# GestaltCogTeam/STEP

Measured on AMD Instinct MI355X. Metric: training windows/sec on PEMS04, horizon-12 MAE parity, 1/2/4/8 MI355X, higher is better.
Workload: dtype f16 (TSFormer Q/K/weights) + bf16 (P, V, GraphWaveNet / graph-learner GEMMs) operands, f32 accumulate

## Files before the change

include/step_hip.h:

```cpp
#ifndef STEP_HIP_H
#define STEP_HIP_H

#include <stdint.h>

#ifdef __cplusplus
extern "C" {
#endif

const char* step_last_error(void);
int step_abi_version(void);

typedef struct StepGemm {
    int M, N, K, batch;
    const void* A; long sam, sak, sab; int a_bf16;
    const void* B; long sbk, sbn, sbb; int b_bf16;
    float* C; long ldc, scn, scb;
    float alpha;
    int accumulate;
    const float* bias; int relu;
    int splitk;
    int a_kblk; long a_kstride;
    int b_kblk; long b_kstride;
    int b_nblk; long b_nstride;
    int c_nblk; long c_nstride;
// ... 8 lines not shown
int step_gemm(const StepGemm* g, void* stream);

#define STEP_ENC_F16 1
#define STEP_ENC_ALWAYS_RESHIFT 2
#define STEP_ENC_RANGE_FLAG 4
#define STEP_ENC_WORKGROUPS(n) (((n) & 0xffff) << 8)
int step_tsformer_encode(const float* series, int S, int L, const void* wpack, long wpack_bytes,
                         int depth, int flags, uint16_t* hidden_bf16, float* hidden_f32, float* last_f32,
                         float* sqnorm_part, float dropout_p, const uint64_t* drop_pool, long pool_words, uint64_t seed,
                         unsigned int* fallback_count, void* stream);
int step_dropout_pool_fill(uint64_t* pool, long words, float dropout_p, uint64_t seed, void* stream);
long step_tsformer_dropout_words(int L, int depth);

int step_pack_long_history(const float* x, int B, int L, int N, int C, int ch, float* out, void* stream);
int step_gather_windows(const float* data, int T, int N, int C, int ch, const long* t0, int B, int L, int H,
                        float* long_series, float* hist, float* fut, void* stream);

long step_knn_workspace_bytes(int B, int N, int F);
int step_knn_graph(const uint16_t* hidden, const float* sqnorm_part, int B, int N, int F, int k_total,
                   float* sim, float* adj, void* work, long work_bytes, void* stream);
int step_topk_mask(const float* sim, int B, int N, int k_total, float* adj, void* work, long work_bytes,
                   void* stream);

typedef struct StepDglParams {
    float *conv1_w, *conv1_b;
    float *conv2_w, *conv2_b;
    float *fc_w, *fc_b;
    float *bn1_w, *bn1_b, *bn1_rm, *bn1_rv;
    float *bn2_w, *bn2_b, *bn2_rm, *bn2_rv;
    float *bn3_w, *bn3_b, *bn3_rm, *bn3_rv;
    float *fc_out_w, *fc_out_b;
    float *fc_cat_w, *fc_cat_b;
    int gemm_bf16;
} StepDglParams;

long step_dgl_global_saved_floats(int N, int T);
long step_dgl_global_work_floats(int N, int T, int backward);
int step_dgl_global_forward(const float* series_nt, int N, int T, const StepDglParams* p, int training,
                            float momentum, float* saved, float* work, float* g, void* stream);
int step_dgl_global_backward(const float* series_nt, int N, int T, const StepDglParams* p, const float* saved,
                             const float* dg, float* work, const StepDglParams* grads, void* stream);
#define STEP_DGL_FRESH_FC_GRAD 16
int step_dgl_global_backward_phase(const float* series_nt, int N, int T, const StepDglParams* p, const float* saved,
                             const float* dg, float* work, const StepDglParams* grads, int phase, void* stream);

typedef struct StepDglShard { int own1; double count1, count2; } StepDglShard;
int step_dgl_global_forward_shard(const float* series_slice, int N, int Ts, const StepDglParams* p, int training, float momentum,
                                  float* saved, float* work, double* sums, float* g, const StepDglShard* shard, int phase,
                                  void* stream);
int step_dgl_global_backward_shard(const float* series_slice, int N, int Ts, const StepDglParams* p, const float* saved,
                                   const float* dg, float* work, const StepDglParams* grads, const StepDglShard* shard, int phase,
                                   void* stream);
long step_dgl_global_offset(int N, int T, int item);

long step_dgl_edges_saved_floats(int B, int N);
long step_dgl_edges_work_floats(int N);
long step_dgl_edges_theta_offset(int N);
int step_dgl_edges_forward(const float* g, int N, int B, const StepDglParams* p, const float* u, uint64_t seed,
                           float temperature, float* saved, float* theta_out, float* adj_out, void* stream);
int step_dgl_edges_forward_keyed(const float* g, int N, int B, const StepDglParams* p, const long* key, uint64_t seed,
                                 float temperature, float* saved, float* theta_out, float* adj_out, void* stream);
int step_dgl_edges_backward(const float* g, int N, int B, const StepDglParams* p, const float* saved,
                            const float* dtheta, const float* dadj, float temperature, float* work,
                            const StepDglParams* grads, float* dg, void* aux_stream, void* stream);
int step_dgl_edges_backward_acc(const float* g, int N, int B, const StepDglParams* p, const float* saved,
                                const float* dtheta, const float* dadj, float temperature, float* work,
                                const StepDglParams* grads, float* dg, int dg_accumulate, void* aux_stream, void* stream);

typedef struct StepGwnetParams {
    float *nodevec1, *nodevec2;
    float *start_w, *start_b;
    float *filter_w[8], *filter_b[8];
    float *gate_w[8], *gate_b[8];
    float *skip_w[8], *skip_b[8];
    float *bn_w[8], *bn_b[8], *bn_rm[8], *bn_rv[8];
    float *gconv_w[8], *gconv_b[8];
    float *fc_his0_w, *fc_his0_b, *fc_his2_w, *fc_his2_b;
    float *end1_w, *end1_b, *end2_w, *end2_b;
    int gemm_bf16;
} StepGwnetParams;

long step_gwnet_saved_floats(int B, int N, int dropout);
long step_gwnet_work_floats(int B, int N, int backward);
long step_gwnet_saved_offset(int B, int N, int dropout, int item, int layer);
int step_gwnet_forward(const float* hist, int B, int N, int Cin, const float* hidden_last, const float* adj,
                       const StepGwnetParams* p, int training, float dropout_p, uint64_t seed, float momentum,
                       float* saved, float* work, float* pred, void* stream);
int step_gwnet_forward_phase(const float* hist, int B, int N, int Cin, const float* hidden_last, const float* adj,
                             const StepGwnetParams* p, int training, float dropout_p, uint64_t seed, float momentum,
                             float* saved, float* work, float* pred, int phase, void* stream);
int step_gwnet_backward(const float* hist, int B, int N, int Cin, const float* hidden_last, const StepGwnetParams* p,
                        const float* saved, float* work, const float* dpred, const StepGwnetParams* grads,
                        float* dadj, int dropout, void* aux_stream, void* leaf_stream, void* stream);

int step_pt_dropout(const float* x, float* y, long n, float p, uint64_t seed, uint32_t site, void* stream);
int step_pt_ffn_hidden_fwd(const float* x, const float* w1, const float* b1, long R, float p, uint64_t seed, uint32_t site,
                           uint16_t* hidden, void* stream);
int step_pt_ffn_hidden_bwd(const float* dy, const float* w2, const uint16_t* hidden, long R, float p, uint16_t* dhidden, void* stream);
int step_pt_colsum_bf16(const uint16_t* x, long rows, int cols, float* out, void* stream);
long step_pt_rows_linear_pack_bytes(int nkc, int nog);
int step_pt_rows_linear_pack(const float* w, long swo, long swi, int nkc, int nog, const float* bias, void* pack, void* stream);
int step_pt_rows_linear(const void* x, int x_bf16, long R, const void* pack, int nkc, int nog, void* y, int y_bf16, int accumulate, void* stream);
int step_pt_layer_pack(const float* wi, const float* bi, const float* wo, const float* bo, const float* w1, const float* b1, const float* w2,
                       const float* b2, void* ffn, void* qkv, void* o, void* da, void* dx, void* stream);
long step_pt_proj_wgrad_ws_floats(long R);
int step_pt_proj_wgrad(const float* x, const uint16_t* dqkv, const float* dov, const uint16_t* a, long R, float* ws, float* dwi, float* dbi, float* dwo,
// ... 141 lines not shown
```

step_amd/_lib.py:

```python
import ctypes
import os

import torch

_HERE = os.path.dirname(os.path.abspath(__file__))
LIB_PATH = os.environ.get("STEP_HIP_LIB") or os.path.join(_HERE, "libstep_hip.so")

_vp, _i, _l, _f, _u64 = ctypes.c_void_p, ctypes.c_int, ctypes.c_long, ctypes.c_float, ctypes.c_uint64


class StepGemm(ctypes.Structure):
    _fields_ = [("M", _i), ("N", _i), ("K", _i), ("batch", _i),
                ("A", _vp), ("sam", _l), ("sak", _l), ("sab", _l), ("a_bf16", _i),
                ("B", _vp), ("sbk", _l), ("sbn", _l), ("sbb", _l), ("b_bf16", _i),
                ("C", _vp), ("ldc", _l), ("scn", _l), ("scb", _l),
                ("alpha", _f), ("accumulate", _i), ("bias", _vp), ("relu", _i), ("splitk", _i),
                ("a_kblk", _i), ("a_kstride", _l), ("b_kblk", _i), ("b_kstride", _l),
                ("b_nblk", _i), ("b_nstride", _l), ("c_nblk", _i), ("c_nstride", _l),
                ("a_kscale", _vp), ("a_kshift", _vp), ("a_kperiod", _i),
                ("batch0", _i), ("sab1", _l), ("sbb1", _l), ("scb1", _l), ("compute_bf16", _i), ("a_rowsum", _vp), ("c_nscale", _vp), ("c_nshift", _vp), ("c_mvec", _vp),
                ("c_nperiod", _i), ("splitk_ws", _vp), ("splitk_ws_floats", _l)]


class StepDglParams(ctypes.Structure):
    NAMES = ["conv1_w", "conv1_b", "conv2_w", "conv2_b", "fc_w", "fc_b",
             "bn1_w", "bn1_b", "bn1_rm", "bn1_rv", "bn2_w", "bn2_b", "bn2_rm", "bn2_rv",
             "bn3_w", "bn3_b", "bn3_rm", "bn3_rv", "fc_out_w", "fc_out_b", "fc_cat_w", "fc_cat_b"]
    _fields_ = [(n, _vp) for n in NAMES] + [("gemm_bf16", _i)]


class StepGwnetParams(ctypes.Structure):
    _fields_ = [("nodevec1", _vp), ("nodevec2", _vp), ("start_w", _vp), ("start_b", _vp),
                ("filter_w", _vp * 8), ("filter_b", _vp * 8), ("gate_w", _vp * 8), ("gate_b", _vp * 8),
                ("skip_w", _vp * 8), ("skip_b", _vp * 8),
                ("bn_w", _vp * 8), ("bn_b", _vp * 8), ("bn_rm", _vp * 8), ("bn_rv", _vp * 8),
                ("gconv_w", _vp * 8), ("gconv_b", _vp * 8),
                ("fc_his0_w", _vp), ("fc_his0_b", _vp), ("fc_his2_w", _vp), ("fc_his2_b", _vp),
                ("end1_w", _vp), ("end1_b", _vp), ("end2_w", _vp), ("end2_b", _vp), ("gemm_bf16", _i)]


_PD = ctypes.POINTER(StepDglParams)


class StepDynState(ctypes.Structure):
    _fields_ = [("seed_xor", ctypes.c_uint64), ("adam_step", ctypes.c_int32), ("lr", _f), ("gsl_coef", _f), ("reserved", _f)]


class StepDglShard(ctypes.Structure):
    _fields_ = [("own1", ctypes.c_int), ("count1", ctypes.c_double), ("count2", ctypes.c_double)]


_PS = ctypes.POINTER(StepDglShard)
_PG = ctypes.POINTER(StepGwnetParams)

_SIGS = {
    "step_last_error": (ctypes.c_char_p, []),
    "step_abi_version": (_i, []),
    "step_gemm": (_i, [ctypes.POINTER(StepGemm), _vp]),
    "step_tsformer_encode": (_i, [_vp, _i, _i, _vp, _l, _i, _i, _vp, _vp, _vp, _vp, _f, _vp, _l, _u64, _vp, _vp]),
    "step_dropout_pool_fill": (_i, [_vp, _l, _f, _u64, _vp]),
    "step_tsformer_dropout_words": (_l, [_i, _i]),
    "step_gather_windows": (_i, [_vp, _i, _i, _i, _i, _vp, _i, _i, _i, _vp, _vp, _vp, _vp]),
    "step_pack_long_history": (_i, [_vp, _i, _i, _i, _i, _i, _vp, _vp]),
    "step_knn_workspace_bytes": (_l, [_i, _i, _i]),
    "step_knn_graph": (_i, [_vp, _vp, _i, _i, _i, _i, _vp, _vp, _vp, _l, _vp]),
    "step_topk_mask": (_i, [_vp, _i, _i, _i, _vp, _vp, _l, _vp]),
    "step_selftest_mfma": (_i, [_vp, _vp]),
    "step_streams_concurrent": (_i, [_vp, _vp, ctypes.POINTER(_i)]),
    "step_dgl_global_saved_floats": (_l, [_i, _i]),
    "step_dgl_global_work_floats": (_l, [_i, _i, _i]),
    "step_dgl_global_forward": (_i, [_vp, _i, _i, _PD, _i, _f, _vp, _vp, _vp, _vp]),
    "step_dgl_global_backward": (_i, [_vp, _i, _i, _PD, _vp, _vp, _vp, _PD, _vp]),
    "step_dgl_global_backward_phase": (_i, [_vp, _i, _i, _PD, _vp, _vp, _vp, _PD, _i, _vp]),
    "step_dgl_global_forward_shard": (_i, [_vp, _i, _i, _PD, _i, _f, _vp, _vp, _vp, _vp, _PS, _i, _vp]),
    "step_dgl_global_backward_shard": (_i, [_vp, _i, _i, _PD, _vp, _vp, _vp, _PD, _PS, _i, _vp]),
    "step_dgl_global_offset": (_l, [_i, _i, _i]),
    "step_dgl_edges_saved_floats": (_l, [_i, _i]),
    "step_dgl_edges_work_floats": (_l, [_i]),
    "step_dgl_edges_theta_offset": (_l, [_i]),
    "step_dgl_edges_forward": (_i, [_vp, _i, _i, _PD, _vp, _u64, _f, _vp, _vp, _vp, _vp]),
    "step_dgl_edges_forward_keyed": (_i, [_vp, _i, _i, _PD, _vp, _u64, _f, _vp, _vp, _vp, _vp]),
    "step_dgl_edges_backward": (_i, [_vp, _i, _i, _PD, _vp, _vp, _vp, _f, _vp, _PD, _vp, _vp, _vp]),
    "step_dgl_edges_backward_acc": (_i, [_vp, _i, _i, _PD, _vp, _vp, _vp, _f, _vp, _PD, _vp, _i, _vp, _vp]),
    "step_gwnet_saved_floats": (_l, [_i, _i, _i]),
    "step_gwnet_work_floats": (_l, [_i, _i, _i]),
    "step_gwnet_saved_offset": (_l, [_i, _i, _i, _i, _i]),
    "step_gwnet_forward": (_i, [_vp, _i, _i, _i, _vp, _vp, _PG, _i, _f, _u64, _f, _vp, _vp, _vp, _vp]),
    "step_gwnet_forward_phase": (_i, [_vp, _i, _i, _i, _vp, _vp, _PG, _i, _f, _u64, _f, _vp, _vp, _vp, _i, _vp]),
    "step_gwnet_backward": (_i, [_vp, _i, _i, _i, _vp, _PG, _vp, _vp, _vp, _PG, _vp, _i, _vp, _vp, _vp]),
    "step_pt_dropout": (_i, [_vp, _vp, _l, _f, _u64, ctypes.c_uint32, _vp]),
    "step_pt_ffn_hidden_fwd": (_i, [_vp, _vp, _vp, _l, _f, _u64, ctypes.c_uint32, _vp, _vp]),
    "step_pt_ffn_hidden_bwd": (_i, [_vp, _vp, _vp, _l, _f, _vp, _vp]),
    "step_pt_colsum_bf16": (_i, [_vp, _l, _i, _vp, _vp]),
    "step_pt_rows_linear_pack_bytes": (_l, [_i, _i]),
    "step_pt_rows_linear_pack": (_i, [_vp, _l, _l, _i, _i, _vp, _vp, _vp]),
    "step_pt_rows_linear": (_i, [_vp, _i, _l, _vp, _i, _i, _vp, _i, _i, _vp]),
    "step_pt_layer_pack": (_i, [_vp] * 14),
    "step_pt_proj_wgrad_ws_floats": (_l, [_l]),
    "step_pt_proj_wgrad": (_i, [_vp, _vp, _vp, _vp, _l, _vp, _vp, _vp, _vp, _vp]),
    "step_pt_ffn_fused_fwd_ln": (_i, [_vp, _l, _vp, _f, _vp, _l, _u64, ctypes.c_uint32, ctypes.c_uint32, _vp, _vp, _vp, _vp, _vp, _vp]),
    "step_pt_rows_linear_ln": (_i, [_vp, _l, _vp, _vp, _f, _u64, ctypes.c_uint32, _vp, _vp, _vp, _vp, _vp, _vp]),
    "step_pt_embed_unmasked_fwd": (_i, [_vp, _vp, _vp, _vp, _vp, _l, _i, _i, _f, _u64, ctypes.c_uint32, _vp, _vp]),
    "step_pt_embed_unmasked_bwd": (_i, [_vp, _vp, _vp, _l, _i, _i, _f, _u64, ctypes.c_uint32, _vp, _vp, _vp, _vp]),
    "step_pt_dec_input_bwd_sums": (_i, [_vp, _l, _i, _i, _f, _u64, ctypes.c_uint32, _vp, _vp, _vp, _vp, _vp]),
    "step_pt_ffn_pack_bytes": (_l, []),
    "step_pt_ffn_wgrad_workgroups": (_l, [_l]),
    "step_pt_ffn_wgrad_ws_floats": (_l, [_l]),
    "step_pt_ffn_pack": (_i, [_vp, _vp, _vp, _vp, _vp, _vp]),
    "step_pt_ffn_fused_fwd": (_i, [_vp, _l, _vp, _f, _vp, _l, _u64, ctypes.c_uint32, _vp, _vp]),
    "step_pt_ffn_fused_bwd_data": (_i, [_vp, _vp, _l, _vp, _f, _vp, _l, _u64, ctypes.c_uint32, _vp, _vp]),
    "step_pt_ffn_fused_bwd_weights": (_i, [_vp, _vp, _l, _vp, _vp, _f, _vp, _l, _u64, ctypes.c_uint32, _vp, _vp, _vp, _vp, _vp]),
    "step_pt_add_layernorm_fwd": (_i, [_vp, _vp, _l, _f, _u64, ctypes.c_uint32, _vp, _vp, _vp, _vp, _vp, _vp]),
    "step_pt_layernorm_bwd_dropout": (_i, [_vp, _vp, _l, _vp, _vp, _vp, _vp, _f, _u64, ctypes.c_uint32, _vp, _vp, _vp, _vp]),
    "step_pt_dropout_relu_mask": (_i, [_vp, _vp, _l, _f, _u64, ctypes.c_uint32, _vp]),
    "step_pt_add_dropout": (_i, [_vp, _vp, _vp, _l, _f, _u64, ctypes.c_uint32, _vp]),
    "step_pt_add_rows": (_i, [_vp, _l, _i, _vp, _vp, _vp]),
    "step_pt_sum_over_seq": (_i, [_vp, _l, _i, _i, _i, _vp, _vp, _vp]),
    "step_pt_token_gather": (_i, [_vp, _l, _i, _vp, _i, _f, _vp, _vp]),
    "step_pt_token_scatter": (_i, [_vp, _l, _i, _vp, _i, _f, _vp, _vp]),
    "step_pt_dec_input": (_i, [_vp, _vp, _vp, _vp, _l, _i, _i, _f, _u64, ctypes.c_uint32, _vp, _vp]),
    "step_pt_dec_input_bwd": (_i, [_vp, _l, _i, _i, _f, _u64, ctypes.c_uint32, _vp, _vp, _vp]),
    "step_pt_layernorm_fwd": (_i, [_vp, _l, _vp, _vp, _vp, _vp, _vp]),
    "step_pt_layernorm_bwd": (_i, [_vp, _vp, _l, _vp, _vp, _vp, _vp, _vp, _vp]),
    "step_pt_attention_fwd": (_i, [_vp, _l, _i, _f, _u64, ctypes.c_uint32, _vp, _vp, _vp]),
    "step_pt_attention_bwd": (_i, [_vp, _vp, _vp, _vp, _l, _i, _f, _u64, ctypes.c_uint32, _vp, _vp]),
    "step_pt_attention_fwd_bf16": (_i, [_vp, _l, _i, _f, _u64, ctypes.c_uint32, _vp, _vp, _vp, _vp, _l, _vp]),
    "step_pt_attention_bwd_bf16": (_i, [_vp, _vp, _vp, _vp, _l, _i, _f, _u64, ctypes.c_uint32, _vp, _vp, _vp]),
    "step_pt_linear_bf16out": (_i, [_vp, _vp, _l, _l, _vp, _l, _i, _i, _vp, _vp]),
    "step_pt_relu_mask": (_i, [_vp, _vp, _l, _vp]),
# ... 122 lines not shown
```

step_amd/csrc/dgl.hip:

```cpp
#include "common.h"
#include "step_internal.h"

namespace {

constexpr int KW = 10;
constexpr int EMB = 100;

template <int CI, int CO, int TPT>
__global__ __launch_bounds__(256) void conv_relu_fwd_kernel(const float* __restrict__ in, const float* __restrict__ w,
                                                            const float* __restrict__ b, const float* __restrict__ in_sc,
                                                            const float* __restrict__ in_sh, float* __restrict__ out,
                                                            float* __restrict__ partial, int Tin, int stat_limit) {
    __shared__ __attribute__((aligned(16))) float ws[CI * KW * CO];
    __shared__ float red[4][2 * CO];
    const int tid = threadIdx.x, n = blockIdx.y;
    const int Tout = Tin - (KW - 1);
    for (int e = tid; e < CI * KW * CO; e += 256) {
        int co = e % CO, k = (e / CO) % KW, ci = e / (CO * KW);
        ws[e] = w[(co * CI + ci) * KW + k];
    }
    __syncthreads();
    const int t0 = (blockIdx.x * 256 + tid) * TPT;
    float acc[CO][TPT];
#pragma unroll
// ... 622 lines not shown
    if (i < n) gpre[i] = shiftdot[i % EMB];
}
__global__ __launch_bounds__(256) void fc_unpermute_kernel(const float* __restrict__ graw, const float* __restrict__ fc_w,
                                                           const float* __restrict__ st2, const float* __restrict__ colsum,
                                                           float* __restrict__ dfc_w, float* __restrict__ dots_o, int T2, int overwrite) {
    __shared__ float red[16][32];
    const int o = blockIdx.y, t = blockIdx.x * 256 + threadIdx.x, tid = threadIdx.x, lane = tid & 63, wave = tid >> 6;
    const float cso = colsum[o];
    float d[32];
#pragma unroll
    for (int i = 0; i < 32; ++i) d[i] = 0.f;
    if (t < T2) {
        const float4* src = (const float4*)(graw + ((long)o * T2 + t) * 16);
        const float4 g0 = src[0], g1 = src[1], g2 = src[2], g3 = src[3];
        const float g[16] = {g0.x, g0.y, g0.z, g0.w, g1.x, g1.y, g1.z, g1.w, g2.x, g2.y, g2.z, g2.w, g3.x, g3.y, g3.z, g3.w};
        float w[16], old[16];
#pragma unroll
        for (int c = 0; c < 16; ++c) { const long idx = ((long)o * 16 + c) * T2 + t; w[c] = fc_w[idx]; old[c] = overwrite ? 0.f : dfc_w[idx]; }
#pragma unroll
        for (int c = 0; c < 16; ++c) {
            dfc_w[((long)o * 16 + c) * T2 + t] = old[c] + st2[c] * g[c] + st2[16 + c] * cso;
            d[2 * c] = w[c] * g[c]; d[2 * c + 1] = w[c] * cso;
        }
    }
#pragma unroll
    for (int i = 0; i < 32; ++i) {
        const float v = row_sum_fast(d[i]);
        if ((lane & 15) == 15) red[4 * wave + (lane >> 4)][i] = v;
    }
    __syncthreads();
    if (tid < 32) {
        float v = 0.f;
#pragma unroll
        for (int r = 0; r < 16; ++r) v += red[r][tid];
        atomicAdd(&dots_o[o * 32 + tid], v);
    }
}
__global__ void dots_reduce_kernel(const float* __restrict__ dots_o, float* __restrict__ dots) {
    const int i = threadIdx.x;
    if (i >= 32) return;
    double a = 0.0;
    for (int o = 0; o < EMB; ++o) a += dots_o[o * 32 + i];
    dots[i] = (float)a;
}

static bool dgl_channels_last(const StepDglParams* p) {
    const char* e = getenv("STEP_DGL_F32_STORAGE");
    return p->gemm_bf16 && !(e && e[0] == '1');
}

static bool dgl_fc_stream() {
    const char* e = getenv("STEP_DGL_FC_STREAM");
    return !(e && e[0] == '0' && e[1] == 0);
}

static bool dgl_legacy_bn_backward() {
    const char* e = getenv("STEP_DGL_LEGACY_BN");
    return e && e[0] == '1';
}

extern "C" long step_dgl_global_saved_floats(int N, int T) {
    long T1 = T - 9, T2 = T - 18;
    return (long)N * 8 * T1 + (long)N * 16 * T2 + (long)N * EMB + 4 * 8 + 4 * 16 + 4 * EMB + (long)EMB * 16 * T2 + 128;
}
static long fc_splitk_ws_floats(int N, int T2) {
    const int splits = step_gemm_auto_splitk(N, EMB, 16 * T2, 1);
    return splits > 1 ? (long)splits * N * EMB + 4 : 0;
}
static long wraw_floats(long T2) {
    const long w = (long)EMB * 16 * T2, pack = dgl_conv2_pack_floats();
    return w > pack ? w : pack;
}
extern "C" long step_dgl_global_work_floats(int N, int T, int backward) {
    long T1 = T - 9, T2 = T - 18;
    long nb1 = (long)N * cdiv(T1, 1024), nb2 = (long)N * cdiv(T2, 1024);
    long part = (nb1 > nb2 ? nb1 : nb2) * 32 + 64;
    if (!backward) return part + dgl_conv2_pack_floats() + 64 + fc_splitk_ws_floats(N, (int)T2);
    return part + (long)N * 16 * T2 + (long)N * 8 * T1 + wraw_floats(T2) + 2L * N * EMB + DGL_SMALL + dgl_conv2_wgrad_scratch_floats(N, (int)T1);
}

static float* saved_wp(float* saved, int N, int T) {
    long T1 = T - 9, T2 = T - 18;
    return saved + (long)N * 8 * T1 + (long)N * 16 * T2 + (long)N * EMB + 4 * 8 + 4 * 16 + 4 * EMB;
}
static void carve_saved(float* saved, int N, int T, float** a1, float** a2, float** gpre, float** st1, float** st2, float** st3) {
    long T1 = T - 9, T2 = T - 18;
    *a1 = saved; saved += (long)N * 8 * T1;
    *a2 = saved; saved += (long)N * 16 * T2;
    *gpre = saved; saved += (long)N * EMB;
    *st1 = saved; saved += 4 * 8;
    *st2 = saved; saved += 4 * 16;
    *st3 = saved;
}

static int dgl_bn_stats(const float* partial, int nblk, int C, double count, const float* gamma, const float* beta, float* rm, float* rv,
                        int training, float momentum, float* stat, double* sums, hipStream_t st) {
    if (nblk < 8192) {
        bn_finalize_kernel<<<C, 256, 0, st>>>(partial, nblk, C, count, gamma, beta, rm, rv, training, momentum, stat);
    } else {
        if (hipMemsetAsync(sums, 0, 2 * C * sizeof(double), st) != hipSuccess) { step_set_error("memset failed"); return STEP_ERR_HIP; }
        bn_sums_sliced_kernel<<<dim3(C, 32), 256, 0, st>>>(partial, nblk, C, sums);
        bn_finalize_sums_kernel<<<1, 64, 0, st>>>(sums, C, count, gamma, beta, rm, rv, training, momentum, stat);
    }
    STEP_LAUNCH_CHECK("bn_stats");
    return STEP_OK;
}
// ... 123 lines not shown
extern "C" int step_dgl_global_backward_shard(const float* series_slice, int N, int Ts, const StepDglParams* p, const float* saved,
                                              const float* dg, float* work, const StepDglParams* grads, const StepDglShard* shard,
                                              int phase, void* stream) {
    const int ph = phase & ~STEP_DGL_FRESH_FC_GRAD;
    STEP_REQUIRE(series_slice && p && saved && dg && work && grads && shard && N > 0 && Ts > 18 && (ph == 1 || ph == 3 || ph == 4),
                 "dgl_global_backward_shard: bad arguments");
    STEP_REQUIRE(p->gemm_bf16 && Ts - 18 >= 128, "dgl_global_backward_shard: needs the bf16 contraction mode and a slice of >= 128 conv2 columns");
    return dgl_global_backward_impl(series_slice, N, Ts, p, saved, dg, work, grads, shard, phase, stream);
}

static int dgl_global_backward_impl(const float* series_nt, int N, int T, const StepDglParams* p, const float* saved, const float* dg,
                                    float* work, const StepDglParams* grads, const StepDglShard* shard, int phase, void* stream) {
    const int fresh_fc = (phase & STEP_DGL_FRESH_FC_GRAD) ? 1 : 0;
    phase &= ~STEP_DGL_FRESH_FC_GRAD;
    const bool do_fc = phase == 0 || phase == 1, do_mid = phase == 0 || phase == 2 || phase == 3, do_tail = phase == 0 || phase == 2 || phase == 4;
    hipStream_t st = (hipStream_t)stream;
    const int T1 = T - 9, T2 = T - 18;
    const long K = 16L * T2;
    float *a1, *a2, *gpre, *st1, *st2, *st3;
    carve_saved((float*)saved, N, T, &a1, &a2, &gpre, &st1, &st2, &st3);
    long nb1 = (long)N * cdiv(T1, 1024), nb2 = (long)N * cdiv(T2, 1024);
    float* partial = work;
    float* d_a2 = work + (nb1 > nb2 ? nb1 : nb2) * 32 + 64;
    float* d_a1 = d_a2 + (long)N * 16 * T2;
    float* wraw = d_a1 + (long)N * 8 * T1;
    float* dgpre = wraw + wraw_floats(T2);
    float* dgpreT = dgpre + (long)N * EMB;
    float* coef = dgpreT + (long)N * EMB;
    float* dots = coef + 256;
    float* graw = coef + 320;
    float* wg_scratch = coef + DGL_SMALL;
    const bool fuse2 = T2 >= 128 && (shard || !dgl_legacy_bn_backward());
    const double count1 = shard ? shard->count1 : (double)N * T1, count2 = shard ? shard->count2 : (double)N * T2;
    if (dgl_channels_last(p)) {
        const float* wp = saved_wp((float*)saved, N, T);
        float* dots_o = coef + 256 + 64 + 1344;
        float* colsum = coef + 128;
        if (do_fc) {
            bn3_relu_bwd_kernel<<<EMB, 256, 0, st>>>(dg, gpre, N, p->bn3_w, st3, grads->bn3_w, grads->bn3_b, grads->fc_b, dgpre, dgpreT, colsum);
            STEP_LAUNCH_CHECK("bn3_bwd");
            StepGemm gm = gemm_desc(EMB, (int)K, N, dgpre, 1, EMB, a2, K, 1, wraw, K);
            gm.b_bf16 = 1;
            gm.compute_bf16 = 1;
            if (dgl_fc_stream() && dgl_fc_stream_wgrad_ok(N)) STEP_TRY(dgl_fc_stream_wgrad(a2, dgpreT, N, EMB, K, wraw, st));
            else STEP_TRY(step_gemm_launch(gm, st));
            if (hipMemsetAsync(dots_o, 0, EMB * 32 * sizeof(float), st) != hipSuccess) { step_set_error("memset failed"); return STEP_ERR_HIP; }
            fc_unpermute_kernel<<<dim3(cdiv(T2, 256), EMB), 256, 0, st>>>(wraw, p->fc_w, st2, colsum, grads->fc_w, dots_o, T2, fresh_fc);
            dots_reduce_kernel<<<1, 64, 0, st>>>(dots_o, dots);
            STEP_LAUNCH_CHECK("fc_unpermute");
        }
        if (do_mid) {
            bn2_fused_coef_kernel<<<1, 64, 0, st>>>(dots, st2, p->bn2_w, count2, grads->bn2_w, grads->bn2_b, coef);
            STEP_LAUNCH_CHECK("bn2_fused_coef");
            StepGemm gm = gemm_desc(N, (int)K, EMB, dgpre, EMB, 1, wp, K, 1, d_a2, K);
            gm.b_bf16 = 1;
            gm.compute_bf16 = 1;
            GemmFused fu = {nullptr, nullptr, a2, coef, st2, 16, T2, GEMM_FUSED_INTERLEAVED};
            STEP_TRY(step_gemm_launch_fused(gm, fu, st));
            STEP_TRY(dgl_conv2_wgrad_cl(d_a2, a1, wg_scratch, graw, N, T1, st));
        }
        if (do_tail) {
            STEP_TRY(dgl_conv2_wgrad_finish(graw, p->conv2_w, st1, p->bn1_w, p->bn1_b, count1, grads->conv2_w, grads->conv2_b, grads->bn1_w,
                                            grads->bn1_b, coef + 64, 1, st));
            STEP_TRY(dgl_conv2_dgrad_cl(d_a2, p->conv2_w, st1, d_a1, N, T1, a1, coef + 64, st1, shard ? shard->own1 : T1, wraw, st));
            STEP_TRY(dgl_conv1_wgrad_cl(d_a1, series_nt, wg_scratch, grads->conv1_w, grads->conv1_b, N, T, st));
        }
        return STEP_OK;
    }
    if (do_fc) {
        float* colsum = coef + 128;
        bn3_relu_bwd_kernel<<<EMB, 256, 0, st>>>(dg, gpre, N, p->bn3_w, st3, grads->bn3_w, grads->bn3_b, grads->fc_b, dgpre, dgpreT, colsum);
        STEP_LAUNCH_CHECK("bn3_bwd");
        {
            StepGemm gm = gemm_desc(EMB, (int)K, N, dgpre, 1, EMB, a2, K, 1, grads->fc_w, K);
            gm.accumulate = fresh_fc ? 0 : 1;
            gm.c_nscale = st2; gm.c_nshift = st2 + 16; gm.c_nperiod = T2; gm.c_mvec = colsum;
            gm.compute_bf16 = p->gemm_bf16;
            if (fuse2) {
                if (hipMemsetAsync(dots, 0, 32 * sizeof(float), st) != hipSuccess) { step_set_error("memset failed"); return STEP_ERR_HIP; }
                GemmFused fu = {p->fc_w, dots, nullptr, nullptr, nullptr, 16, T2};
                STEP_TRY(step_gemm_launch_fused(gm, fu, st));
            } else {
                STEP_TRY(step_gemm_launch(gm, st));
            }
        }
    }
    if (!do_mid && !do_tail) return STEP_OK;
    if (do_mid) {
        StepGemm gm = gemm_desc(N, (int)K, EMB, dgpreT, 1, N, p->fc_w, K, 1, d_a2, K);
        if (p->gemm_bf16 || fuse2) { gm.A = dgpre; gm.sam = EMB; gm.sak = 1; }
        gm.compute_bf16 = p->gemm_bf16;
        if (fuse2) {
            bn2_fused_coef_kernel<<<1, 64, 0, st>>>(dots, st2, p->bn2_w, count2, grads->bn2_w, grads->bn2_b, coef);
            STEP_LAUNCH_CHECK("bn2_fused_coef");
            GemmFused fu = {nullptr, nullptr, a2, coef, st2, 16, T2};
            STEP_TRY(step_gemm_launch_fused(gm, fu, st));
        } else {
            STEP_TRY(step_gemm_launch(gm, st));
        }
    }
    if (do_mid && !fuse2) {
        dim3 grid(cdiv(T2, 1024), 16, N);
        bn_bwd_reduce_kernel<16><<<grid, 256, 0, st>>>(d_a2, a2, st2, T2, partial);
        STEP_LAUNCH_CHECK("bn2_bwd_reduce");
        bn_bwd_finalize_kernel<<<16, 256, 0, st>>>(partial, (int)nb2, 16, (double)N * T2, p->bn2_w, st2, grads->bn2_w, grads->bn2_b, coef);
        STEP_LAUNCH_CHECK("bn2_bwd_finalize");
        bn_bwd_apply_kernel<16><<<grid, 256, 0, st>>>(d_a2, a2, st2, coef, T2);
        STEP_LAUNCH_CHECK("bn2_bwd_apply");
    }
    const bool fuse1 = p->gemm_bf16 && (shard || !dgl_legacy_bn_backward());
    if (fuse1) {
// ... 150 lines not shown
```

step_amd/csrc/dgl_fc_stream.hip:

```cpp
#include "common.h"
#include "step_internal.h"
#include "lds_dma.h"
#include <stdlib.h>

namespace {

template <int N>
__device__ __forceinline__ void fs_wait_vm() {
    static_assert(N >= 0 && N <= 63, "vmcnt");
    if constexpr (N == 0) asm volatile("s_waitcnt vmcnt(0)" ::: "memory");
    else if constexpr (N == 5) asm volatile("s_waitcnt vmcnt(5)" ::: "memory");
    else if constexpr (N == 6) asm volatile("s_waitcnt vmcnt(6)" ::: "memory");
    else if constexpr (N == 20) asm volatile("s_waitcnt vmcnt(20)" ::: "memory");
    else if constexpr (N == 40) asm volatile("s_waitcnt vmcnt(40)" ::: "memory");
    else static_assert(N == 0, "add the case");
}
__device__ __forceinline__ void fs_barrier() {
    __builtin_amdgcn_s_barrier();
    asm volatile("" ::: "memory");
}

constexpr int FS_TM = 320, FS_KS = 64, FS_ROWB = FS_KS * 2, FS_WROWS = 104, FS_RING = 3, FS_WAVES = 10;
constexpr int FS_STAGE = (FS_TM + FS_WROWS) * FS_ROWB;
static_assert(FS_RING * FS_STAGE <= 160 * 1024, "forward ring");
static_assert(FS_TM / 8 == 4 * FS_WAVES, "four a2h row groups per wave");

__global__ __launch_bounds__(FS_WAVES * 64) void fc_stream_fwd_kernel(const uint16_t* __restrict__ A, const uint16_t* __restrict__ W, int N, int O,
                                                                       long K, int per, float* __restrict__ out, long range_stride, int atomic) {
    extern __shared__ __attribute__((aligned(16))) char fs_lds[];
    const int tid = threadIdx.x, lane = tid & 63, wave = __builtin_amdgcn_readfirstlane(tid >> 6);
    const int s = blockIdx.x, row0 = blockIdx.y * FS_TM;
    const int ksteps = (int)((K + FS_KS - 1) / FS_KS);
    const int step0 = s * per;
    const int nstep = min(ksteps - step0, per);
    const int rp = wave % 5, cp = wave / 5;
    f32x16 acc[4];
#pragma unroll
    for (int t = 0; t < 4; ++t)
#pragma unroll
        for (int e = 0; e < 16; ++e) acc[t][e] = 0.f;
    const uint32_t lds0 = (uint32_t)(uintptr_t)(__attribute__((address_space(3))) char*)fs_lds;
    const int pc = (lane & 7) ^ (lane >> 3);
    const uint16_t* src[6];
#pragma unroll
    for (int j = 0; j < 4; ++j) {
        const int row = min(row0 + (wave * 4 + j) * 8 + (lane >> 3), N - 1);
        src[j] = A + (long)row * K;
    }
    src[4] = W + (long)min(wave * 8 + (lane >> 3), O - 1) * K;
    src[5] = W + (long)min((10 + wave) * 8 + (lane >> 3), O - 1) * K;
    const bool six = wave < 3;
    auto issue = [&](int step, int buf) {
        const long k0 = (long)(step0 + step) * FS_KS;
        const long off = k0 + (k0 + pc * 8 < K ? pc * 8 : 0);
        const uint32_t base = lds0 + (uint32_t)(buf * FS_STAGE);
#pragma unroll
        for (int j = 0; j < 4; ++j) lds_dma_1k(src[j] + off, base + (uint32_t)((wave * 4 + j) * 1024));
        lds_dma_1k(src[4] + off, base + (uint32_t)(FS_TM * FS_ROWB + wave * 1024));
        if (six) lds_dma_1k(src[5] + off, base + (uint32_t)(FS_TM * FS_ROWB + (10 + wave) * 1024));
    };
    if (nstep > 0) {
        const int r = lane & 31, h = lane >> 5;
        const int wr0 = min(cp * 64 + r, O - 1), wr1 = min(cp * 64 + 32 + r, O - 1);
        const int offa0 = (rp * 64 + r) * FS_ROWB, offa1 = offa0 + 32 * FS_ROWB;
        const int offb0 = (FS_TM + wr0) * FS_ROWB, offb1 = (FS_TM + wr1) * FS_ROWB;
        const int xa = r & 7, xb0 = wr0 & 7, xb1 = wr1 & 7;
        issue(0, 0);
// ... 99 lines not shown
            const int o = min(i / (WG_TN / 2), O - 1), n = (i % (WG_TN / 2)) * 2;
            v0[j] = dT[(long)o * N + min(n, N - 1)];
            v1[j] = dT[(long)o * N + min(n + 1, N - 1)];
        }
#pragma unroll
        for (int j = 0; j < PER; ++j) {
            const int i = tid + (c * PER + j) * WG_THREADS;
            const int o = i / (WG_TN / 2), n = (i % (WG_TN / 2)) * 2;
            *(uint32_t*)(dlds + o * WG_DPITCH + n * 2) = pack_bf16x2((o < O && n < N) ? v0[j] : 0.f, (o < O && n + 1 < N) ? v1[j] : 0.f);
        }
    }
    asm volatile("s_waitcnt lgkmcnt(0)" ::: "memory");
    fs_barrier();
    if (producer) {
        for (int i = 0; i < ntile; ++i) {
            if (i + 2 < ntile) fs_wait_vm<2 * (WG_TN / 16)>();
            else if (i + 1 < ntile) fs_wait_vm<WG_TN / 16>();
            else fs_wait_vm<0>();
            fs_barrier();
            if (i + 3 < ntile) issue(i + 3, (i + 3) % WG_RING);
        }
        return;
    }
    const int r = lane & 31, h = lane >> 5;
    const int orow = min(wave * 32 + r, O - 1);
    const char* pa = dlds + orow * WG_DPITCH + h * 16;
    const int troff = (8 * h + ((lane & 15) >> 2)) * WG_ROWB + (16 * ((lane >> 4) & 1) + 4 * (lane & 3)) * 2;
    bf16x8 afr[WG_TN / 16];
#pragma unroll
    for (int kb = 0; kb < WG_TN / 16; ++kb) afr[kb] = *(const bf16x8*)(pa + kb * 32);
    f32x16 acc0, acc1;
    for (int i = 0; i < ntile; ++i) {
        fs_barrier();
        const char* pb = ring + (i % WG_RING) * WG_STAGE + troff;
#pragma unroll
        for (int e = 0; e < 16; ++e) { acc0[e] = 0.f; acc1[e] = 0.f; }
#pragma unroll
        for (int kb2 = 0; kb2 < WG_TN / 32; ++kb2) {
            const char* q0 = pb + kb2 * 32 * WG_ROWB;
            const u32x2 l0 = fs_read_tr(q0), h0 = fs_read_tr(q0 + 4 * WG_ROWB);
            const u32x2 l1 = fs_read_tr(q0 + 16 * WG_ROWB), h1 = fs_read_tr(q0 + 20 * WG_ROWB);
            const u32x4 b0 = {l0[0], l0[1], h0[0], h0[1]}, b1 = {l1[0], l1[1], h1[0], h1[1]};
            acc0 = __builtin_amdgcn_mfma_f32_32x32x16_bf16(afr[2 * kb2], __builtin_bit_cast(bf16x8, b0), acc0, 0, 0, 0);
            acc1 = __builtin_amdgcn_mfma_f32_32x32x16_bf16(afr[2 * kb2 + 1], __builtin_bit_cast(bf16x8, b1), acc1, 0, 0, 0);
        }
        const long col = (long)(tile0 + i) * WG_CT + r;
        const int ob = wave * 32 + 4 * h;
        if (col < K) {
#pragma unroll
            for (int e = 0; e < 16; ++e) {
                const int o = ob + 8 * (e >> 2) + (e & 3);
                if (o < O) G[(long)o * K + col] = acc0[e] + acc1[e];
            }
        }
    }
}

int env_int(const char* name, int dflt) {
    const char* e = getenv(name);
    return e && e[0] ? atoi(e) : dflt;
}

}

bool dgl_fc_stream_wgrad_ok(int N) { return N <= WG_TN; }

constexpr int FS_RANGES = 96;
int dgl_fc_stream_fwd(const void* a2h, const void* wp, int N, int O, long K, float* gpre, float* ws, long ws_floats, hipStream_t st) {
    STEP_REQUIRE(a2h && wp && gpre && N > 0 && O > 0 && O <= FS_WROWS && K > 0 && K % 16 == 0, "dgl_fc_stream_fwd: bad arguments");
    const int ksteps = (int)((K + FS_KS - 1) / FS_KS);
    const long mn = (long)N * O;
    long ranges = (ws && (((uintptr_t)ws) & 15) == 0) ? ws_floats / mn : 1;
    const int want = env_int("STEP_DGL_FC_STREAM_RANGES", FS_RANGES);
    if (ranges > want) ranges = want;
    if (ranges > ksteps) ranges = ksteps;
    if (ranges < 1) ranges = 1;
    const int per = (ksteps + (int)ranges - 1) / (int)ranges;
    const int used = (ksteps + per - 1) / per;
    STEP_TRY(step_raise_lds_once((const void*)fc_stream_fwd_kernel, 160 * 1024, "dgl_fc_stream_fwd"));
    const dim3 grid(used, cdiv(N, FS_TM));
    const bool direct = used == 1;
    fc_stream_fwd_kernel<<<grid, FS_WAVES * 64, FS_RING * FS_STAGE, st>>>((const uint16_t*)a2h, (const uint16_t*)wp, N, O, K, per, direct ? gpre : ws,
                                                                         direct ? 0 : mn, direct ? 1 : 0);
    STEP_LAUNCH_CHECK("dgl_fc_stream_fwd");
    if (!direct) {
        const int chunk = 16;
        fc_stream_reduce_kernel<<<dim3((unsigned)((mn + 255) / 256), (unsigned)cdiv(used, chunk)), 256, 0, st>>>(ws, used, chunk, mn, gpre);
        STEP_LAUNCH_CHECK("dgl_fc_stream_fwd(reduce)");
    }
    return STEP_OK;
}

int dgl_fc_stream_wgrad(const void* a2h, const float* dgpreT, int N, int O, long K, float* G, hipStream_t st) {
    STEP_REQUIRE(a2h && dgpreT && G && N > 0 && N <= WG_TN && O > 0 && O <= WG_OROWS && K > 0 && K % 16 == 0, "dgl_fc_stream_wgrad: bad arguments");
    const int tiles = (int)((K + WG_CT - 1) / WG_CT);
    int groups = env_int("STEP_DGL_FC_STREAM_WGROUPS", 256);
    if (groups > tiles) groups = tiles;
    if (groups < 1) groups = 1;
    const int per = (tiles + groups - 1) / groups;
    STEP_TRY(step_raise_lds_once((const void*)fc_stream_wgrad_kernel, 160 * 1024, "dgl_fc_stream_wgrad"));
    fc_stream_wgrad_kernel<<<(tiles + per - 1) / per, WG_THREADS, WG_DBYTES + WG_RING * WG_STAGE, st>>>((const uint16_t*)a2h, dgpreT, N, O, K, per, G);
    STEP_LAUNCH_CHECK("dgl_fc_stream_wgrad");
    return STEP_OK;
}
```

step_amd/csrc/step_internal.h:

```cpp
#pragma once
#include <hip/hip_runtime.h>
#include <vector>
#include "../../include/step_hip.h"

enum { GEMM_FUSED_INTERLEAVED = 1, GEMM_FUSED_FFN_FWD = 2, GEMM_FUSED_MASKNZ = 4, GEMM_FUSED_BF16OUT = 8 };
struct GemmFused {
    const float* dotw; float* dots;
    const float* bnx; const float* bncoef; const float* bnstat;
    int channels, period;
    int flags;
    const float* ffn_bias; const void* maskx; float p; unsigned seed_lo, seed_hi, site;
};

struct GemmKSeg { long a_off, b_off, a_bs, b_bs; int a_rs, b_rs; };
constexpr int GEMM_KSEG_MAX = 128;
int step_gemm_segmented_launch(StepGemm g, const GemmKSeg* ktab, int ktab_per, hipStream_t st);

int step_gemm_launch(StepGemm g, hipStream_t st);
int step_gemm_auto_splitk(int M, int N, int K, int batch);
int step_gemm_launch_fused(StepGemm g, const GemmFused& fused, hipStream_t st);
int step_gemm_bf16_launch(StepGemm g, hipStream_t st, const GemmFused* fused = nullptr);
int step_gemm_f32_fast_launch(StepGemm g, hipStream_t st, const GemmFused* fused = nullptr);

static inline StepGemm gemm_desc(int M, int N, int K, const float* A, long sam, long sak, const float* B, long sbk,
                                 long sbn, float* C, long ldc) {
    StepGemm g;
    memset(&g, 0, sizeof(g));
    g.M = M; g.N = N; g.K = K; g.batch = 1;
    g.A = A; g.sam = sam; g.sak = sak;
    g.B = B; g.sbk = sbk; g.sbn = sbn;
    g.C = C; g.ldc = ldc; g.scn = 1;
    g.alpha = 1.f; g.splitk = 1;
    return g;
}

int step_gemm_rowsum_separate(StepGemm* g, hipStream_t st);
int dgl_conv2_fwd_mfma(const float* a1, const float* w, const float* b, const float* sc, const float* sh, float* a2, float* partial,
                       int N, int T1, int* nblk, hipStream_t st);
int dgl_conv2_dgrad_mfma(const float* dz, const float* w, float* din, int N, int T1, const float* bnx, const float* coef, const float* stat,
                         int own, hipStream_t st);
int dgl_conv2_wgrad_xhat_mfma(const float* dz, const float* a1, const float* stat1, float* scratch, float* graw, int N, int T1, hipStream_t st);
int dgl_conv2_wgrad_finish(const float* graw, const float* w, const float* stat1, const float* gamma1, const float* beta1, double count,
                           float* dw, float* db, float* dgamma1, float* dbeta1, float* coef1, int raw, hipStream_t st);
int dgl_conv1_fwd_cl(const float* x, const float* w, const float* b, void* a1h, float* partial, int N, int T, int stat_limit, int* nblk,
                     hipStream_t st);
long dgl_conv2_pack_floats();
int dgl_conv2_fwd_cl(const void* a1h, const float* w, const float* b, const float* sc, const float* sh, void* a2h, float* partial, int N,
                     int T1, int* nblk, float* pack, hipStream_t st);
int dgl_conv2_dgrad_cl(const void* dz2h, const float* w, const float* sc, void* dz1h, int N, int T1, const void* a1h, const float* coef,
                       const float* stat, int own, float* pack, hipStream_t st);
int dgl_conv2_wgrad_cl(const void* dz2h, const void* a1h, float* scratch, float* graw, int N, int T1, hipStream_t st);
int dgl_conv1_wgrad_cl(const void* dz1h, const float* x, float* scratch, float* dw, float* db, int N, int T, hipStream_t st);
long dgl_conv2_wgrad_scratch_floats(int N, int T1);
int dgl_conv2_wgrad_mfma(const float* dz, const float* a1, const float* sc, const float* sh, float* scratch, float* dw, float* db, int N,
                         int T1, hipStream_t st);
int dgl_conv1_wgrad_mfma(const float* dz, const float* x, float* scratch, float* dw, float* db, int N, int T, hipStream_t st);
int dgl_fc_stream_fwd(const void* a2h, const void* wp, int N, int O, long K, float* gpre, float* ws, long ws_floats, hipStream_t st);
bool dgl_fc_stream_wgrad_ok(int N);
int dgl_fc_stream_wgrad(const void* a2h, const float* dgpreT, int N, int O, long K, float* G, hipStream_t st);
int step_colsum_launch(const float* x, long rows, int cols, long ld, float* out, hipStream_t st);

struct AuxLane {
    hipStream_t main, aux;
    bool on;
    int next = 0, base = 0;
    AuxLane(hipStream_t m, hipStream_t a, int base_ = 0) : main(m), aux(a), on(a != nullptr && a != m), base(base_) {}
    static hipEvent_t event(int k) {
        thread_local std::vector<hipEvent_t> pool[16];
        int dev = 0;
        (void)hipGetDevice(&dev);
        std::vector<hipEvent_t>& v = pool[dev & 15];
        while ((int)v.size() <= k) {
            hipEvent_t e;
            if (hipEventCreateWithFlags(&e, hipEventDisableTiming) != hipSuccess) return nullptr;
            v.push_back(e);
        }
        return v[k];
    }
    hipStream_t fork() {
        if (!on) return main;
        hipEvent_t e = event(base + (next++ & 63));
        if (!e || hipEventRecord(e, main) != hipSuccess || hipStreamWaitEvent(aux, e, 0) != hipSuccess) { on = false; return main; }
        return aux;
    }
    hipEvent_t mark() {
        if (!on) return nullptr;
        hipEvent_t e = event(base + (next++ & 63));
        if (!e || hipEventRecord(e, main) != hipSuccess) { on = false; return nullptr; }
        return e;
    }
    hipStream_t after(hipEvent_t e) {
        if (!on || !e) return main;
        if (hipStreamWaitEvent(aux, e, 0) != hipSuccess) { on = false; return main; }
        return aux;
    }
    hipEvent_t done() {
        if (!on) return nullptr;
        hipEvent_t e = event(base + (next++ & 63));
        if (!e || hipEventRecord(e, aux) != hipSuccess) return nullptr;
        return e;
    }
    int wait_done(hipEvent_t e) {
        if (!on) return STEP_OK;
        if (!e) return join();
        if (hipStreamWaitEvent(main, e, 0) != hipSuccess) { step_set_error("backward: stream join failed"); return STEP_ERR_HIP; }
        return STEP_OK;
    }
    int join() {
        if (!on) return STEP_OK;
        hipEvent_t e = event(base + (next++ & 63));
        if (!e || hipEventRecord(e, aux) != hipSuccess || hipStreamWaitEvent(main, e, 0) != hipSuccess) {
            step_set_error("backward: stream join failed");
// ... 6 lines not shown
```

Measured before the change: 2427.

## Add streaming DMA-pipelined kernel for DGL fc input-gradient with fused BN/ReLU epilogue

Adds a dedicated kernel for the graph-learner fc layer's input gradient. One producer wave streams A and W tiles into a ring of LDS buffers via DMA while math waves hold dgpre fragments in registers, run bf16 MFMAs, apply the BN2/ReLU backward correction in-place in LDS, and write bf16 dz2 out. It replaces the generic fused GEMM when N fits in three row tiles and the stream path is enabled, which it is by default. The aim is to remove the generic GEMM's overhead on this tall-K, small-N/O shape and overlap loads with compute, at the cost of more specialised code with fixed limits (O<=100) and large LDS use.

Measured after the change: 2470 (median of 6 runs). 1.02x the previous value.

```diff
diff --git a/include/step_hip.h b/include/step_hip.h
--- a/include/step_hip.h
+++ b/include/step_hip.h
@@ -84,6 +84,10 @@
                                    const float* dg, float* work, const StepDglParams* grads, const StepDglShard* shard, int phase,
                                    void* stream);
 long step_dgl_global_offset(int N, int T, int item);
+
+int step_dgl_fc_dgrad(const float* dgpre, const void* wp, const void* a2h, const float* coef, const float* st2, int N, long K,
+                      void* dz2h, void* stream);
+long step_dgl_fc_dgrad_streams(int N, long K);
 
 long step_dgl_edges_saved_floats(int B, int N);
 long step_dgl_edges_work_floats(int N);
diff --git a/step_amd/_lib.py b/step_amd/_lib.py
--- a/step_amd/_lib.py
+++ b/step_amd/_lib.py
@@ -75,6 +75,8 @@
     "step_dgl_global_forward_shard": (_i, [_vp, _i, _i, _PD, _i, _f, _vp, _vp, _vp, _vp, _PS, _i, _vp]),
     "step_dgl_global_backward_shard": (_i, [_vp, _i, _i, _PD, _vp, _vp, _vp, _PD, _PS, _i, _vp]),
     "step_dgl_global_offset": (_l, [_i, _i, _i]),
+    "step_dgl_fc_dgrad": (_i, [_vp, _vp, _vp, _vp, _vp, _i, _l, _vp, _vp]),
+    "step_dgl_fc_dgrad_streams": (_l, [_i, _l]),
     "step_dgl_edges_saved_floats": (_l, [_i, _i]),
     "step_dgl_edges_work_floats": (_l, [_i]),
     "step_dgl_edges_theta_offset": (_l, [_i]),
diff --git a/step_amd/csrc/dgl.hip b/step_amd/csrc/dgl.hip
--- a/step_amd/csrc/dgl.hip
+++ b/step_amd/csrc/dgl.hip
@@ -698,6 +698,25 @@
 static bool dgl_fc_stream() {
     const char* e = getenv("STEP_DGL_FC_STREAM");
     return !(e && e[0] == '0' && e[1] == 0);
+}
+
+static int dgl_fc_dgrad(const float* dgpre, const void* wp, const void* a2h, const float* coef, const float* st2, int N, long K, void* dz2h,
+                        hipStream_t st) {
+    if (dgl_fc_stream() && dgl_fc_stream_dgrad_ok(N, K)) return dgl_fc_stream_dgrad(dgpre, wp, a2h, coef, st2, N, EMB, K, dz2h, st);
+    StepGemm gm = gemm_desc(N, (int)K, EMB, dgpre, EMB, 1, (const float*)wp, K, 1, (float*)dz2h, K);
+    gm.b_bf16 = 1;
+    gm.compute_bf16 = 1;
+    GemmFused fu = {nullptr, nullptr, (const float*)a2h, coef, st2, 16, (int)(K / 16), GEMM_FUSED_INTERLEAVED};
+    return step_gemm_launch_fused(gm, fu, st);
+}
+
+extern "C" long step_dgl_fc_dgrad_streams(int N, long K) { return dgl_fc_stream() && dgl_fc_stream_dgrad_ok(N, K) ? 1 : 0; }
+
+extern "C" int step_dgl_fc_dgrad(const float* dgpre, const void* wp, const void* a2h, const float* coef, const float* st2, int N, long K,
+                                 void* dz2h, void* stream) {
+    STEP_REQUIRE(dgpre && wp && a2h && coef && st2 && dz2h && N > 0 && K > 0 && K % 16 == 0 && K <= 0x7fffffffL, "dgl_fc_dgrad: bad arguments");
+    STEP_REQUIRE(((((uintptr_t)dgpre) | ((uintptr_t)wp) | ((uintptr_t)a2h) | ((uintptr_t)dz2h)) & 15) == 0, "dgl_fc_dgrad: buffers must be 16-byte aligned");
+    return dgl_fc_dgrad(dgpre, wp, a2h, coef, st2, N, K, dz2h, (hipStream_t)stream);
 }
 
 static bool dgl_legacy_bn_backward() {
@@ -927,11 +946,7 @@
         if (do_mid) {
             bn2_fused_coef_kernel<<<1, 64, 0, st>>>(dots, st2, p->bn2_w, count2, grads->bn2_w, grads->bn2_b, coef);
             STEP_LAUNCH_CHECK("bn2_fused_coef");
-            StepGemm gm = gemm_desc(N, (int)K, EMB, dgpre, EMB, 1, wp, K, 1, d_a2, K);
-            gm.b_bf16 = 1;
-            gm.compute_bf16 = 1;
-            GemmFused fu = {nullptr, nullptr, a2, coef, st2, 16, T2, GEMM_FUSED_INTERLEAVED};
-            STEP_TRY(step_gemm_launch_fused(gm, fu, st));
+            STEP_TRY(dgl_fc_dgrad(dgpre, wp, a2, coef, st2, N, K, d_a2, st));
             STEP_TRY(dgl_conv2_wgrad_cl(d_a2, a1, wg_scratch, graw, N, T1, st));
         }
         if (do_tail) {
diff --git a/step_amd/csrc/dgl_fc_stream.hip b/step_amd/csrc/dgl_fc_stream.hip
--- a/step_amd/csrc/dgl_fc_stream.hip
+++ b/step_amd/csrc/dgl_fc_stream.hip
@@ -13,6 +13,7 @@
     else if constexpr (N == 6) asm volatile("s_waitcnt vmcnt(6)" ::: "memory");
     else if constexpr (N == 20) asm volatile("s_waitcnt vmcnt(20)" ::: "memory");
     else if constexpr (N == 40) asm volatile("s_waitcnt vmcnt(40)" ::: "memory");
+    else if constexpr (N == 53) asm volatile("s_waitcnt vmcnt(53)" ::: "memory");
     else static_assert(N == 0, "add the case");
 }
 __device__ __forceinline__ void fs_barrier() {
@@ -218,6 +219,128 @@
                 const int o = ob + 8 * (e >> 2) + (e & 3);
                 if (o < O) G[(long)o * K + col] = acc0[e] + acc1[e];
             }
+        }
+    }
+}
+
+constexpr int DG_TM = FS_TM, DG_CT = FS_KS, DG_ROWB = FS_ROWB, DG_WROWS = FS_WROWS, DG_RING = FS_RING, DG_STAGE = FS_STAGE;
+constexpr int DG_MATH_WAVES = DG_TM / 64, DG_THREADS = (DG_MATH_WAVES + 1) * 64, DG_OMAX = 100, DG_KB = (DG_OMAX + 15) / 16;
+constexpr int DG_LOADS = (DG_TM + DG_WROWS) / 8;
+static_assert(DG_LOADS <= 63 && DG_WROWS % 8 == 0 && DG_WROWS >= 16 * (DG_KB - 1) + 8 && DG_RING * DG_STAGE <= 160 * 1024, "input-gradient stage");
+
+__global__ __launch_bounds__(DG_THREADS) void fc_stream_dgrad_kernel(const float* __restrict__ D, const uint16_t* __restrict__ W,
+                                                                     const uint16_t* __restrict__ A, const float* __restrict__ coef,
+                                                                     const float* __restrict__ st2, int N, int O, long K, int per, int rtiles,
+                                                                     uint16_t* __restrict__ out) {
+    extern __shared__ __attribute__((aligned(16))) char fs_lds[];
+    const int tid = threadIdx.x, lane = tid & 63, wave = __builtin_amdgcn_readfirstlane(tid >> 6);
+    const int rt = blockIdx.x % rtiles, s = blockIdx.x / rtiles;
+    const int row0 = rt * DG_TM;
+    const int tiles = (int)((K + DG_CT - 1) / DG_CT);
+    const int tile0 = s * per;
+    const int ntile = min(tiles - tile0, per);
+    if (ntile <= 0) return;
+    if (wave == DG_MATH_WAVES) {
+        const uint32_t lds0 = (uint32_t)(uintptr_t)(__attribute__((address_space(3))) char*)fs_lds;
+        const int pca = (lane & 7) ^ (lane >> 3), pcw = (lane & 7) ^ (((lane >> 4) & 1) << 2);
+        auto issue = [&](int tile, int buf) {
+            const long c0 = (long)(tile0 + tile) * DG_CT;
+            const long offa = c0 + (c0 + pca * 8 < K ? pca * 8 : 0), offw = c0 + (c0 + pcw * 8 < K ? pcw * 8 : 0);
+            const uint32_t base = lds0 + (uint32_t)(buf * DG_STAGE);
+#pragma unroll
+            for (int j = 0; j < DG_TM / 8; ++j)
+                lds_dma_1k(A + (long)min(row0 + j * 8 + (lane >> 3), N - 1) * K + offa, base + (uint32_t)(j * 1024));
+#pragma unroll
+            for (int j = 0; j < DG_WROWS / 8; ++j)
+                lds_dma_1k(W + (long)min(j * 8 + (lane >> 3), O - 1) * K + offw, base + (uint32_t)(DG_TM * DG_ROWB + j * 1024));
+        };
+        issue(0, 0);
+        if (ntile > 1) issue(1, 1);
+        for (int i = 0; i < ntile; ++i) {
+            if (i + 1 < ntile) fs_wait_vm<DG_LOADS>(); else fs_wait_vm<0>();
+            fs_barrier();
+            if (i + 2 < ntile) issue(i + 2, (i + 2) % DG_RING);
+        }
+        return;
+    }
+    const int r = lane & 31, h = lane >> 5;
+    bf16x8 afr[2][DG_KB];
+#pragma unroll
+    for (int t2 = 0; t2 < 2; ++t2) {
+        const float* d = D + (long)min(row0 + wave * 64 + t2 * 32 + r, N - 1) * O;
+#pragma unroll
+        for (int kb = 0; kb < DG_KB; ++kb) {
+            float v[8];
+#pragma unroll
+            for (int j = 0; j < 8; ++j) {
+                const int o = kb * 16 + 8 * h + j;
+                const float x = d[min(o, O - 1)];
+                v[j] = o < O ? x : 0.f;
+            }
+            afr[t2][kb] = pack8(v);
+        }
+    }
+    const int c = lane & 15;
+    const float km1 = coef[32 + c] * coef[c], km2 = coef[32 + c] * coef[16 + c] * st2[48 + c], mu = st2[32 + c];
+    const int q = (lane & 15) >> 2, qb = (q >> 1) & 1;
+    int trw[2];
+#pragma unroll
+    for (int j = 0; j < 2; ++j) trw[j] = DG_TM * DG_ROWB + q * DG_ROWB + (j ^ qb) * 64 + ((lane >> 4) & 1) * 32 + (lane & 3) * 8;
+    int xoff[4][2];
+#pragma unroll
+    for (int e3 = 0; e3 < 4; ++e3)
+#pragma unroll
+        for (int j = 0; j < 2; ++j) {
+            const int r7 = e3 + 4 * h;
+            xoff[e3][j] = (wave * 64 + r7) * DG_ROWB + (((j * 4 + (r >> 3)) ^ r7) << 4) + (r & 7) * 2;
+        }
+    const int pc = (lane & 7) ^ (lane >> 3);
+    for (int i = 0; i < ntile; ++i) {
+        fs_barrier();
+        char* buf = fs_lds + (i % DG_RING) * DG_STAGE;
+        f32x16 acc[4];
+#pragma unroll
+        for (int t = 0; t < 4; ++t)
+#pragma unroll
+            for (int e = 0; e < 16; ++e) acc[t][e] = 0.f;
+#pragma unroll
+        for (int kb = 0; kb < DG_KB; ++kb) {
+            const int rowb = 16 * kb + 8 * h < DG_WROWS ? 16 * kb + 8 * h : 16 * kb;
+            bf16x8 b[2];
+#pragma unroll
+            for (int j = 0; j < 2; ++j) {
+                const char* p = buf + rowb * DG_ROWB + trw[j];
+                const u32x2 lo = fs_read_tr(p), hi = fs_read_tr(p + 4 * DG_ROWB);
+                const u32x4 t = {lo[0], lo[1], hi[0], hi[1]};
+                b[j] = __builtin_bit_cast(bf16x8, t);
+            }
+            acc[0] = __builtin_amdgcn_mfma_f32_32x32x16_bf16(afr[0][kb], b[0], acc[0], 0, 0, 0);
+            acc[1] = __builtin_amdgcn_mfma_f32_32x32x16_bf16(afr[0][kb], b[1], acc[1], 0, 0, 0);
+            acc[2] = __builtin_amdgcn_mfma_f32_32x32x16_bf16(afr[1][kb], b[0], acc[2], 0, 0, 0);
+            acc[3] = __builtin_amdgcn_mfma_f32_32x32x16_bf16(afr[1][kb], b[1], acc[3], 0, 0, 0);
+        }
+#pragma unroll
+        for (int t = 0; t < 4; ++t) {
+            uint16_t xb[16];
+#pragma unroll
+            for (int e = 0; e < 16; ++e) xb[e] = *(const uint16_t*)(buf + ((t >> 1) * 32 + 8 * (e >> 2)) * DG_ROWB + xoff[e & 3][t & 1]);
+#pragma unroll
+            for (int e = 0; e < 16; ++e) {
+                const float x = __uint_as_float((uint32_t)xb[e] << 16);
+                const float v = acc[t][e];
+                const float o = x > 0.f ? v - km1 - (x - mu) * km2 : 0.f;
+                *(uint16_t*)(buf + ((t >> 1) * 32 + 8 * (e >> 2)) * DG_ROWB + xoff[e & 3][t & 1]) = __builtin_bit_cast(uint16_t, (__bf16)o);
+            }
+        }
+        asm volatile("s_waitcnt lgkmcnt(0)" ::: "memory");
+        const long col = (long)(tile0 + i) * DG_CT + pc * 8;
+        uint4 piece[8];
+#pragma unroll
+        for (int it = 0; it < 8; ++it) piece[it] = *(const uint4*)(buf + (wave * 64 + it * 8 + (lane >> 3)) * DG_ROWB + (lane & 7) * 16);
+#pragma unroll
+        for (int it = 0; it < 8; ++it) {
+            const int row = row0 + wave * 64 + it * 8 + (lane >> 3);
+            if (row < N && col < K) *(uint4*)(out + (long)row * K + col) = piece[it];
         }
     }
 }
@@ -269,3 +392,25 @@
     STEP_LAUNCH_CHECK("dgl_fc_stream_wgrad");
     return STEP_OK;
 }
+
+constexpr int DG_MAX_RTILES = 3;
+bool dgl_fc_stream_dgrad_ok(int N, long K) { return N > 0 && N <= DG_MAX_RTILES * DG_TM && K > 0; }
+
+constexpr int DG_GROUPS = 256;
+int dgl_fc_stream_dgrad(const float* dgpre, const void* wp, const void* a2h, const float* coef, const float* st2, int N, int O, long K,
+                        void* dz2h, hipStream_t st) {
+    STEP_REQUIRE(dgpre && wp && a2h && coef && st2 && dz2h && N > 0 && O > 0 && O <= DG_OMAX && K > 0 && K % 16 == 0,
+                 "dgl_fc_stream_dgrad: bad arguments");
+    STEP_REQUIRE(((((uintptr_t)wp) | ((uintptr_t)a2h) | ((uintptr_t)dz2h)) & 15) == 0, "dgl_fc_stream_dgrad: wp, a2h and dz2h must be 16-byte aligned");
+    const int tiles = (int)((K + DG_CT - 1) / DG_CT), rtiles = cdiv(N, DG_TM);
+    int ranges = env_int("STEP_DGL_FC_STREAM_DGROUPS", DG_GROUPS) / rtiles;
+    if (ranges > tiles) ranges = tiles;
+    if (ranges < 1) ranges = 1;
+    const int per = (tiles + ranges - 1) / ranges;
+    const int used = (tiles + per - 1) / per;
+    STEP_TRY(step_raise_lds_once((const void*)fc_stream_dgrad_kernel, 160 * 1024, "dgl_fc_stream_dgrad"));
+    fc_stream_dgrad_kernel<<<used * rtiles, DG_THREADS, DG_RING * DG_STAGE, st>>>(dgpre, (const uint16_t*)wp, (const uint16_t*)a2h, coef, st2, N, O, K, per,
+                                                                                 rtiles, (uint16_t*)dz2h);
+    STEP_LAUNCH_CHECK("dgl_fc_stream_dgrad");
+    return STEP_OK;
+}
diff --git a/step_amd/csrc/step_internal.h b/step_amd/csrc/step_internal.h
--- a/step_amd/csrc/step_internal.h
+++ b/step_amd/csrc/step_internal.h
@@ -58,6 +58,9 @@
 int dgl_fc_stream_fwd(const void* a2h, const void* wp, int N, int O, long K, float* gpre, float* ws, long ws_floats, hipStream_t st);
 bool dgl_fc_stream_wgrad_ok(int N);
 int dgl_fc_stream_wgrad(const void* a2h, const float* dgpreT, int N, int O, long K, float* G, hipStream_t st);
+bool dgl_fc_stream_dgrad_ok(int N, long K);
+int dgl_fc_stream_dgrad(const float* dgpre, const void* wp, const void* a2h, const float* coef, const float* st2, int N, int O, long K,
+                        void* dz2h, hipStream_t st);
 int step_colsum_launch(const float* x, long rows, int cols, long ld, float* out, hipStream_t st);
 
 struct AuxLane {
```
